# dfm/tinygp

Hardware: AMD Instinct MI355X
Metric: GP log_probability evals/sec + Cholesky TFLOP/s (fp64), N=16,384 (higher is better)
Workload: dtype f64; 1 GPU; c2: 1.5^2 ExpSquared(2.5), 1-D X, N=16384, fp64, diag=0.01, constant-density synthetic inputs (SURVEY 8d), dense Cholesky + tri-solve; n=16384, d=1, parallelism=single, nb_outer=1024

## Files before the change

### tinygp_amd/csrc/capi.hip

```cpp
#include <cmath>
#include <cstdlib>
#include <chrono>
#include <cstring>
#include <string>

#include "tgp_common.h"
#define CHAIN_HD __host__ __device__
#include "chain_tasks.h"
#define TILE_HD
#include "tile_order.h"

namespace tgp {

static thread_local std::string g_error;

void set_error(const char* fmt, ...) {
  char buf[1024];
  va_list ap;
  va_start(ap, fmt);
  vsnprintf(buf, sizeof(buf), fmt, ap);
  va_end(ap);
  g_error = buf;
}

// ... 155 lines not shown
  TGP_HIP_TRY(hipStreamCreateWithPriority(&ctx->update_stream, hipStreamNonBlocking, hi));
  TGP_HIP_TRY(hipStreamCreateWithPriority(&ctx->asm_stream, hipStreamNonBlocking, lo));
  TGP_HIP_TRY(hipEventCreateWithFlags(&ctx->ev_asm, hipEventDisableTiming));
  TGP_HIP_TRY(hipEventCreateWithFlags(&ctx->ev_d, hipEventDisableTiming));
  TGP_HIP_TRY(hipEventCreateWithFlags(&ctx->ev_e, hipEventDisableTiming));
  TGP_HIP_TRY(hipEventCreateWithFlags(&ctx->ev_f, hipEventDisableTiming));
  TGP_HIP_TRY(hipEventCreateWithFlags(&ctx->ev_g1, hipEventDisableTiming));
  TGP_HIP_TRY(hipEventCreateWithFlags(&ctx->ev_g2, hipEventDisableTiming));
  TGP_HIP_TRY(hipEventCreateWithFlags(&ctx->ev_h, hipEventDisableTiming));
  TGP_HIP_TRY(hipEventCreateWithFlags(&ctx->ev_i, hipEventDisableTiming));
  TGP_HIP_TRY(hipEventCreateWithFlags(&ctx->ev_j, hipEventDisableTiming));
  TGP_HIP_TRY(hipEventCreateWithFlags(&ctx->ev_c, hipEventDisableTiming));
  TGP_HIP_TRY(hipEventCreateWithFlags(&ctx->ev_join, hipEventDisableTiming));
  TGP_HIP_TRY(hipEventCreateWithFlags(&ctx->ev_a, hipEventDisableTiming));
  TGP_HIP_TRY(hipEventCreateWithFlags(&ctx->ev_b, hipEventDisableTiming));
  TGP_HIP_TRY(hipMalloc(&ctx->d_scal, 16 * sizeof(double)));
  TGP_HIP_TRY(hipMalloc(&ctx->d_info, sizeof(int32_t)));
  TGP_HIP_TRY(hipMalloc(&ctx->d_step_flag, 64));
  TGP_HIP_TRY(hipMemset(ctx->d_step_flag, 0, 64));
  TGP_HIP_TRY(hipMalloc(&ctx->d_chain_flags, size_t(tgp::CHAIN_MAX_ROW_TILES) * 64 * sizeof(uint32_t)));
  TGP_HIP_TRY(hipMemset(ctx->d_chain_flags, 0, size_t(tgp::CHAIN_MAX_ROW_TILES) * 64 * sizeof(uint32_t)));
  TGP_HIP_TRY(hipMalloc(&ctx->d_chain_ticket, 4096));
  TGP_HIP_TRY(hipMemset(ctx->d_chain_ticket, 0, 4096));
  TGP_HIP_TRY(hipMalloc(&ctx->d_chain_red, size_t(2) * CHAIN_MAX_ROW_TILES * sizeof(double)));
  hipDeviceProp_t prop;
  TGP_HIP_TRY(hipGetDeviceProperties(&prop, device));
  ctx->cus = prop.multiProcessorCount;
  *out = ctx;
  return TGP_OK;
}

int tgp_ctx_destroy(tgp_ctx* ctx) {
// ... 17 lines not shown
    hipStreamSynchronize(ctx->asm_stream);
    hipStreamDestroy(ctx->asm_stream);
  }
  if (ctx->ev_asm) hipEventDestroy(ctx->ev_asm);
  if (ctx->ev_d) hipEventDestroy(ctx->ev_d);
  if (ctx->ev_e) hipEventDestroy(ctx->ev_e);
  if (ctx->ev_f) hipEventDestroy(ctx->ev_f);
  if (ctx->ev_g1) hipEventDestroy(ctx->ev_g1);
  if (ctx->ev_g2) hipEventDestroy(ctx->ev_g2);
  if (ctx->ev_h) hipEventDestroy(ctx->ev_h);
  if (ctx->ev_i) hipEventDestroy(ctx->ev_i);
  if (ctx->ev_j) hipEventDestroy(ctx->ev_j);
  for (auto e : ctx->ev_pool) hipEventDestroy(e);
  if (ctx->ev_a) hipEventDestroy(ctx->ev_a);
  if (ctx->ev_b) hipEventDestroy(ctx->ev_b);
  if (ctx->d_scal) hipFree(ctx->d_scal);
  if (ctx->d_info) hipFree(ctx->d_info);
  if (ctx->d_step_flag) hipFree(ctx->d_step_flag);
  if (ctx->d_chain_flags) hipFree(ctx->d_chain_flags);
  if (ctx->d_chain_ticket) hipFree(ctx->d_chain_ticket);
  if (ctx->d_chain_red) hipFree(ctx->d_chain_red);
  if (ctx->d_chain_stamps) hipFree(ctx->d_chain_stamps);
  for (auto& kv : ctx->chain_tables)
    if (kv.second.dev) hipFree(kv.second.dev);
  if (ctx->d_dinv) hipFree(ctx->d_dinv);
  if (ctx->d_work) hipFree(ctx->d_work);
  if (ctx->d_gemm_ws) hipFree(ctx->d_gemm_ws);
  if (ctx->d_gemm_prefix_count) hipFree(ctx->d_gemm_prefix_count);
  if (ctx->panel_stream) hipStreamDestroy(ctx->panel_stream);
  if (ctx->own_stream && ctx->stream) hipStreamDestroy(ctx->stream);
  delete ctx;
  return TGP_OK;
// ... 398 lines not shown
    tgp_ctx* ctx = s->ctx;
    for (hipStream_t q : {ctx->asm_stream, ctx->panel_stream, ctx->update_stream, ctx->solve_stream, ctx->stream})
      if (q) (void)hipStreamSynchronize(q);
    (void)hipGetLastError();
    ctx->asm_pending = false;
    ctx->deferred_asm = nullptr;
    ctx->ev_used = 0;
    ctx->timeout_retries++;
    const int64_t keep = ctx->chain_kernel;
    ctx->chain_kernel = 0;
    st = factor_body(s, prog, nops, cov_host, info, fused, resid_host, logprob);
    ctx->chain_kernel = keep;
  }
  if (st < 0) {
    tgp_ctx* ctx = s->ctx;
    ctx->asm_pending = false;
    ctx->deferred_asm = nullptr;
    ctx->ev_used = 0;
    s->factored = false;
    for (hipStream_t q : {ctx->asm_stream, ctx->panel_stream, ctx->update_stream, ctx->solve_stream,
                          ctx->stream})
      if (q) (void)hipStreamSynchronize(q);
    (void)hipGetLastError();
  }
  return st;
}

static int factor_body(tgp_solver* s, const tgp_kop* prog, int nops, const void* cov_host,
                       int32_t* info, int fused, const void* resid_host, double* logprob) {
  tgp_ctx* ctx = s->ctx;
// ... 6 lines not shown
  TGP_ARG_CHECK(s->has_prog || cov_host != nullptr, "factor needs a kernel program or a covariance");
  s->winv_valid = false;
  const auto host0 = std::chrono::steady_clock::now();
  const size_t es = esize(s->dtype);
  hipEvent_t e0 = nullptr, e1 = nullptr, e2 = nullptr;
  const bool prof = ctx->profile != 0;
  if (prof) {
    TGP_HIP_TRY(hipEventCreate(&e0));
    TGP_HIP_TRY(hipEventCreate(&e1));
    TGP_HIP_TRY(hipEventCreate(&e2));
    TGP_HIP_TRY(hipEventRecord(e0, ctx->stream));
  }
  int status = dispatch(s->dtype, [&](auto tag) {
    using T = decltype(tag);
    T* A = (T*)s->A;
    if (fused) {
      if (resid_host) {
        TGP_TRY(upload_vec(s, s->vec, resid_host));
      } else {
        TGP_ARG_CHECK(s->has_resid, "no resident residual: call tgp_solver_set_resid first");
        TGP_HIP_TRY(hipMemcpyAsync(s->vec, s->resid, size_t(s->npad) * es, hipMemcpyDeviceToDevice,
                                   ctx->stream));
      }
    }
    if (cov_host != nullptr) {
      TGP_TRY(solver_scratch(s, size_t(s->n) * s->n * es));
      TGP_HIP_TRY(hipMemcpyAsync(s->scratch, cov_host, size_t(s->n) * s->n * es,
                                 hipMemcpyHostToDevice, ctx->stream));
      TGP_TRY(launch_set_lower_from_rowmajor<T>(ctx, s->n, s->npad, (const T*)s->scratch, A, s->npad));
    } else {
      TGP_TRY(assemble_lower<T>(ctx, s->kp, s->n, s->d, (const T*)s->X, (const T*)s->diag, A, s->npad));
    }
    if (prof) TGP_HIP_TRY(hipEventRecord(e1, ctx->stream));
    int32_t inf = 0;
    ctx->defer_join = ctx->late_join != 0;
    ctx->join_deferred = false;
    reductions_begin(ctx, s->npad, fused != 0);
    int st = potrf<T>(ctx, s->npad, A, s->npad, (T*)s->dinv, &inf, fused ? (T*)s->vec : (T*)nullptr);
    ctx->defer_join = false;
    const bool reduce = reductions_end(ctx);
    if (st < 0) return st;
    s->info = inf;
    if (prof) TGP_HIP_TRY(hipEventRecord(e2, ctx->stream));
    if (reduce) {
      TGP_TRY(launch_sum_log_diag<T>(ctx, s->n, A, s->npad, 1));
      if (fused) TGP_TRY(launch_sum_squares<T>(ctx, s->n, (const T*)s->vec, 0));
    }
    return TGP_OK;
  });
  if (status < 0) return status;
  double two[2] = {0, 0};
  int32_t inf_late = 0;
  const bool late = ctx->join_deferred;
  ctx->join_deferred = false;
  TGP_HIP_TRY(hipMemcpyAsync(two, ctx->d_scal, 2 * sizeof(double), hipMemcpyDeviceToHost, ctx->stream));
  if (late) TGP_HIP_TRY(hipMemcpyAsync(&inf_late, ctx->d_info, sizeof(int32_t), hipMemcpyDeviceToHost, ctx->stream));
  TGP_HIP_TRY(hipStreamSynchronize(ctx->stream));
  if (late) {
    if (inf_late == INT32_MIN) {
      tgp::set_error("potrf: a device-side hand-off did not arrive within poll_timeout_ms (a lost or starved chain launch)");
      if (prof) { hipEventDestroy(e0); hipEventDestroy(e1); hipEventDestroy(e2); }
      return TGP_E_TIMEOUT;
    }
    s->info = inf_late;
  }
  s->ms[5] = std::chrono::duration<double, std::milli>(ctx->submitted - host0).count();
  s->logdet_half = two[1];
  if (fused && logprob)
    *logprob = -0.5 * two[0] - (s->logdet_half + 0.5 * double(s->n) * std::log(2.0 * M_PI));
  if (prof) {
    float a = 0, b = 0;
    TGP_HIP_TRY(hipEventElapsedTime(&a, e0, e1));
// ... 563 lines not shown
```

### tinygp_amd/csrc/chol.hip

```cpp
#include <algorithm>
#include <atomic>
#include <functional>
#include <type_traits>

#include <thread>

#include "tgp_common.h"
#define CHAIN_HD __host__ __device__
#include "chain_tasks.h"

namespace tgp {

namespace {

typedef double d4 __attribute__((ext_vector_type(4)));
typedef float f4 __attribute__((ext_vector_type(4)));

template <typename T> struct Mfma;
template <> struct Mfma<double> {
  using acc_t = d4;
  static __device__ __forceinline__ acc_t mma(double a, double b, acc_t c) {
    return __builtin_amdgcn_mfma_f64_16x16x4f64(a, b, c, 0, 0, 0);
  }
  static __device__ __forceinline__ int drow(int lane, int r) { return (lane >> 4) + 4 * r; }
// ... 58 lines not shown
#ifdef TGP_POTF2_STAMPS
__device__ long long g_potf2_stamps[64];
#define POTF2_STAMP(i) do { if (threadIdx.x == 0) g_potf2_stamps[i] = __builtin_readcyclecounter(); } while (0)
#else
#define POTF2_STAMP(i) do {} while (0)
#endif

__device__ void potf2_prefix_wait(const int32_t* count, int32_t target, int32_t* info);

template <typename T, bool FOLD>
__global__ __launch_bounds__(512) __attribute__((amdgpu_waves_per_eu(4, 4))) void potf2_kernel(T* __restrict__ A, int64_t ld,
                                                    T* __restrict__ dinv,
                                                    int32_t* __restrict__ info,
                                                    int32_t pivot_base,
                                                    const T* __restrict__ Xp, int64_t ldx,
                                                    const int32_t* __restrict__ wait_count, int32_t wait_target) {
  __shared__ __attribute__((aligned(16))) T S[36 * 256];
  __shared__ T Rs[2 * 16];
  __shared__ T Dg[256];
  if (wait_count != nullptr) {
    if (threadIdx.x == 0) potf2_prefix_wait(wait_count, wait_target, info);
    __syncthreads();
  }
#include "potf2_body.inc"
}

constexpr int32_t STEP_TIMEOUT = INT32_MIN;

__device__ long long g_poll_limit = 400000000LL;
struct PollClock {
  long long t0 = 0;
  __device__ __forceinline__ bool expired(long spin) {
    if ((spin & 255) != 255) return false;
    const long long now = (long long)__builtin_amdgcn_s_memrealtime();
// ... 276 lines not shown
    }
    if (lane == 0) __builtin_amdgcn_fence(__ATOMIC_ACQUIRE, "agent");
  }
  __syncthreads();
}

__device__ __forceinline__ void chain_publish(uint32_t* word, uint32_t value, int32_t* colcnt = nullptr) {
  asm volatile("s_waitcnt vmcnt(0)" ::: "memory");
  __syncthreads();
  if (threadIdx.x == 0) {
    __hip_atomic_store(word, value, __ATOMIC_RELAXED, __HIP_MEMORY_SCOPE_AGENT);
    if (colcnt != nullptr) __hip_atomic_fetch_add(colcnt, 1, __ATOMIC_RELAXED, __HIP_MEMORY_SCOPE_AGENT);
  }
}

__device__ void potf2_prefix_wait(const int32_t* count, int32_t target, int32_t* info) {
  PollClock clk;
  for (unsigned spin = 0;; ++spin) {
    if (__hip_atomic_load(count, __ATOMIC_RELAXED, __HIP_MEMORY_SCOPE_AGENT) >= target) break;
    __builtin_amdgcn_s_sleep(8);
    if ((spin & 255) == 255 && (clk.expired(spin) || poisoned(info))) {
      atomicExch(info, STEP_TIMEOUT);
      break;
    }
  }
  __builtin_amdgcn_fence(__ATOMIC_ACQUIRE, "agent");
}

__global__ __launch_bounds__(64) void chain_poll_kernel(const int32_t* __restrict__ count, int32_t target,
                                                        int32_t* __restrict__ info) {
  if (threadIdx.x != 0) return;
  PollClock clk;
  for (unsigned spin = 0;; ++spin) {
    if (__hip_atomic_load(count, __ATOMIC_RELAXED, __HIP_MEMORY_SCOPE_AGENT) >= target) break;
    __builtin_amdgcn_s_sleep(16);
    if ((spin & 255) == 255 && (clk.expired(spin) || poisoned(info))) {
      atomicExch(info, STEP_TIMEOUT);
      break;
    }
  }
}

template <typename T, int PARTS>
__device__ __forceinline__ void chain_update_full(const ChainArgs<T>& q, T* S, int i, int c, int k, int part) {
  static_assert(PARTS == 1 || PARTS == 4 || PARTS == 8, "whole tile, row quarters or row eighths");
  using M = Mfma<T>;
  using acc_t = typename M::acc_t;
  typedef T T2 __attribute__((ext_vector_type(2)));
  const int tid = threadIdx.x, lane = tid & 63;
// ... 1566 lines not shown
    if ((spin & 63) != 63) continue;
    const double ms = std::chrono::duration<double, std::milli>(std::chrono::steady_clock::now() - t0).count();
    if (ms > budget_ms) break;
    if (ms > 50.0) std::this_thread::sleep_for(std::chrono::microseconds(200));
  }
  if (ctx->rescue_stream == nullptr) TGP_HIP_TRY(hipStreamCreateWithFlags(&ctx->rescue_stream, hipStreamNonBlocking));
  for (int c = 0; c < CHAIN_FLAG_LD; ++c)
    (void)hipStreamWriteValue32(ctx->rescue_stream, ctx->d_chain_ticket + CHAIN_COLCNT_OFF + c, 0x7fffffffu, 0);
  for (hipStream_t q : {ctx->rescue_stream, ctx->asm_stream, ctx->panel_stream, ctx->update_stream, ctx->solve_stream, ctx->stream})
    if (q) (void)hipStreamSynchronize(q);
  (void)hipGetLastError();
  set_error("potrf: the followers of a chain launch were still waiting after %.0f ms (stream wait-values released by the host)", budget_ms);
  return TGP_E_TIMEOUT;
}

template <typename T>
int launch_potf2(tgp_ctx* ctx, hipStream_t st, T* A, int64_t ld, T* dinv, int32_t* info,
                 int32_t pivot_base, const T* Xp, int64_t ldx) {
  if (ctx->trace) {
    trace_push(ctx, 1, st, trace_off(ctx, A), trace_off(ctx, Xp), ld);
    return TGP_OK;
  }
  const int32_t* wc = ctx->potf2_wait_counter;
  const int32_t wt = (int32_t)ctx->potf2_wait_target;
  ctx->potf2_wait_counter = nullptr;
  if (Xp != nullptr)
    hipLaunchKernelGGL((potf2_kernel<T, true>), dim3(1), dim3(512), 0, st, A, ld, dinv, info, pivot_base, Xp, ldx, wc, wt);
  else
    hipLaunchKernelGGL((potf2_kernel<T, false>), dim3(1), dim3(512), 0, st, A, ld, dinv, info, pivot_base, Xp, ldx, wc, wt);
  TGP_HIP_TRY(hipGetLastError());
  return TGP_OK;
}

template <typename T>
int launch_trsm(tgp_ctx* ctx, hipStream_t st, int64_t m, const T* L, int64_t ldl, const T* dinv,
                T* B, int64_t ldb) {
  if (m == 0) return TGP_OK;
  TGP_ARG_CHECK(m % 16 == 0, "trsm: m must be a multiple of 16");
  if (ctx->trace) {
    trace_push(ctx, 2, st, trace_off(ctx, L), trace_off(ctx, B), m, ldl);
    return TGP_OK;
  }
  hipLaunchKernelGGL((trsm_kernel<T>), dim3((unsigned)((m + 63) / 64)), dim3(256), 0, st, m, L,
                     ldl, dinv, B, ldb);
  TGP_HIP_TRY(hipGetLastError());
// ... 20 lines not shown
  TGP_HIP_TRY(hipGetLastError());
  return TGP_OK;
}

template <typename T>
ChainPolicy chain_policy(const tgp_ctx* ctx) {
  if (sizeof(T) != 8 || ctx->chain_batch <= 1) return ChainPolicy{1, 1, 2, 0};
  return ChainPolicy{(int)ctx->chain_batch, (int)ctx->chain_batch_lag, (int)ctx->chain_batch_rowlag, (int)ctx->chain_batch_minrows};
}

template <typename T>
int launch_chain(tgp_ctx* ctx, hipStream_t st, T* A0, int64_t ld, T* dinv0, int64_t pivot_base, int64_t R,
                 int64_t nblk, int64_t cb, int64_t ce, bool head_done, hipEvent_t counters_ready, T* y0, bool fprev) {
  TGP_ARG_CHECK(R >= 1 && R <= CHAIN_MAX_ROW_TILES && cb >= 0 && cb < ce && ce <= nblk && nblk <= CHAIN_FLAG_LD && nblk <= R,
                "chain: bad panel shape (R=%lld, columns [%lld, %lld))", (long long)R, (long long)cb, (long long)ce);
  if (cb == 0 && !head_done) {
    TGP_TRY(launch_potf2<T>(ctx, st, A0, ld, dinv0, ctx->d_info, (int32_t)pivot_base));
    if (!ctx->trace) TGP_TRY(run_deferred_asm(ctx, st));
  }
  if (ctx->chain_polls_pending) {
    TGP_TRY(st_wait(ctx, st, ctx->ev_f));
    ctx->chain_polls_pending = false;
  }
  const int fwd = y0 != nullptr ? 1 : 0;
  int red = 0;
  if (fwd != 0 && ctx->chain_red_total > 0 && ctx->chain_red_total <= CHAIN_MAX_ROW_TILES && pivot_base % TILE == 0) {
    red = 1;
    ctx->chain_red_written += ce - cb;
    if (pivot_base / TILE + ce == ctx->chain_red_total && ctx->chain_red_written == ctx->chain_red_total) {
      red = 2;
      ctx->reductions_done = true;
    }
  }
  if (ctx->trace) {
    if (counters_ready != nullptr) TGP_TRY(ev_record(ctx, counters_ready, st));
    trace_push(ctx, 11, st, trace_off(ctx, A0), ld, R, cb, ce, nblk, fwd, red);
    return TGP_OK;
  }
// ... 29 lines not shown
  q.launch = (int32_t)ctx->chain_launches++;
  q.fast_update = (int32_t)ctx->chain_fast_update;
  q.tasks = found->second.dev;
  q.y = y0;
  q.fgs = CHAIN_FWD_GROUP;
  q.fprev = fprev ? 1 : 0;
  q.red = red != 0 ? ctx->d_chain_red : nullptr;
  q.scal = red != 0 ? ctx->d_scal : nullptr;
  q.red_total = red == 2 ? (int32_t)ctx->chain_red_total : 0;
  if (ctx->chain_stamps != 0 && ctx->chain_stamp_base + tasks <= CHAIN_STAMP_TASKS) {
    if (ctx->d_chain_stamps == nullptr)
      TGP_HIP_TRY(hipMalloc((void**)&ctx->d_chain_stamps, size_t(CHAIN_STAMP_TASKS) * 16 * sizeof(long long)));
    q.stamps = ctx->d_chain_stamps + ctx->chain_stamp_base * 16;
    ctx->chain_stamp_base += tasks;
  }
  TGP_HIP_TRY(hipMemsetAsync(ctx->d_chain_ticket, 0, size_t(CHAIN_TICKET_WORDS) * sizeof(int32_t), st));
  if (counters_ready != nullptr) TGP_TRY(ev_record(ctx, counters_ready, st));
  const size_t dyn = ctx->chain_lds_pad > 0 ? size_t(ctx->chain_lds_pad) + (sizeof(T) == 4 ? 36 * 256 * 4 : 0) : 0;
  hipLaunchKernelGGL((chain_kernel<T>), dim3((unsigned)tasks), dim3(512), dyn, st, q);
  TGP_HIP_TRY(hipGetLastError());
  return TGP_OK;
}

int launch_chain_poll(tgp_ctx* ctx, hipStream_t st, const void* A0, int64_t ld, int64_t R, int64_t c, bool first_external) {
  if (ctx->trace) {
    trace_push(ctx, 12, st, trace_off(ctx, static_cast<const double*>(A0)), ld, c);
    return TGP_OK;
  }
  const int32_t target = (int32_t)(R - c - ((c == 0 && first_external) ? 1 : 0));
  int32_t* count = ctx->d_chain_ticket + CHAIN_COLCNT_OFF + c;
  if (ctx->chain_polls == 3 && ctx->can_wait_value) {
// ... 190 lines not shown
  if (n == 0) return TGP_OK;
  ctx->potf2_wait_counter = nullptr;
  ctx->prefix_hint_cols = 0;
  ctx->prefix_hint_counter = nullptr;
  ctx->reserve_hint = 0;
  hipStream_t S0 = ctx->stream, S1 = ctx->panel_stream;
  if (ctx->solve_on_update == 0 && y != nullptr) TGP_TRY(ensure_solve_stream(ctx));
  hipStream_t S2 = ctx->solve_on_update != 0 ? ctx->update_stream : ctx->solve_stream;
  if (y != nullptr) {
    TGP_TRY(ev_record(ctx, ctx->ev_c, S0));
    TGP_TRY(st_wait(ctx, S2, ctx->ev_c));
  }
  int64_t NB = ctx->nb_outer;
  if (NB < TILE) NB = TILE;
  NB = NB / TILE * TILE;
  if (!ctx->trace) TGP_HIP_TRY(hipMemsetAsync(ctx->d_info, 0, sizeof(int32_t), S0));
  ctx->chain_stamp_base = 0;
  ctx->chain_launches = 0;
  ctx->chain_polls_pending = false;
  const bool prof_on = ctx->profile != 0 && !ctx->trace;
  std::vector<ProfSpan> spans;
  ctx->ev_used = 0;
  hipEvent_t prof_t0 = nullptr;
  const bool span_dump = prof_on && getenv("TGP_SPAN_DUMP") != nullptr;
  if (prof_on) {
    TGP_TRY(prof_event(ctx, &prof_t0));
    TGP_HIP_TRY(hipEventRecord(prof_t0, S0));
  }

  auto potf2_at = [&](hipStream_t st, int64_t j0, bool pend) -> int {
    return panel_potf2<T>(ctx, st, A, ld, dinv, 0, j0, pend);
// ... 33 lines not shown
    const int64_t rem = n - k0;
    int64_t w = NB;
    if (k0 == 0 && ctx->nb_first >= TILE) w = ctx->nb_first / TILE * TILE;
    if (ctx->nb_wide_rows > 0 && k0 > 0 && rem >= ctx->nb_wide_rows) w = 2 * NB;
    if (ctx->chain_kernel != 0 && rem <= ctx->chain_full_rows && rem / TILE <= 64) w = rem;
    return rem < w ? rem : w;
  };
  bool all_chain = ctx->chain_kernel != 0;
  for (int64_t k0 = 0; k0 < n && all_chain; k0 += width(k0))
    all_chain = width(k0) / TILE <= CHAIN_FLAG_LD && (n - k0) / TILE <= CHAIN_MAX_ROW_TILES;
  ctx->chain_fwd_now = y != nullptr && ctx->chain_fwd_tasks != 0 && all_chain;
  auto chain_of_panel = [&](hipStream_t st, int64_t k0, int64_t w) -> int {
    const int64_t sp = ctx->chain_sub_panel / TILE * TILE;
    if (sp >= TILE && sp < w && w % sp == 0 && n - k0 > w && n - k0 >= ctx->chain_sub_min_rows) {
      for (int64_t o = 0; o < w; o += sp) {
        if (o > 0) TGP_TRY(potf2_at(st, k0 + o, false));
        TGP_TRY(panel(st, k0 + o, sp, true, 0, no_mid));
        const int64_t c0 = k0 + o + sp;
        if (c0 < k0 + w)
          TGP_TRY(trailing(st, n - c0, k0 + w - c0, sp, A + (k0 + o) * ld + c0, A + c0 * ld + c0, (int)ctx->chain_sub_role));
      }
      return TGP_OK;
    }
    return panel(st, k0, w, true, 0, no_mid);
  };
  const bool la = ctx->lookahead != 0 && S1 != nullptr;
  if (la && ctx->chain_kernel != 0 && ctx->chain_merged != 0) {
    std::vector<int64_t> s0;
    for (int64_t k0 = 0; k0 < n; k0 += width(k0)) s0.push_back(k0);
    s0.push_back(n);
    const int64_t P = (int64_t)s0.size() - 1;
// ... 5 lines not shown
      TGP_TRY(run_deferred_asm(ctx, nullptr));
    } else {
    TGP_TRY(ev_record(ctx, ctx->ev_a, S0));
    TGP_TRY(st_wait(ctx, S1, ctx->ev_a));
    TGP_TRY(panel(S1, 0, s0[1] - s0[0], false, 0, no_mid));
    TGP_TRY(run_deferred_asm(ctx, nullptr));
    TGP_TRY(ev_record(ctx, ev_chain[0], S1));
    for (int64_t p = 0; p + 1 < P; ++p) {
      const int64_t kb = s0[p + 1] - s0[p], next = s0[p + 1], wn = s0[p + 2] - s0[p + 1], mt = n - next;
      const T* Pp = A + s0[p] * ld + next;
      T* C = A + next * ld + next;
      TGP_TRY(st_wait(ctx, S0, ev_chain[p & 1]));
      if (p == 0 && asm_side) TGP_TRY(st_wait(ctx, S0, ctx->ev_asm));
      const bool prefix = wn < mt && ctx->chain_polls != 0;
      int32_t* counter = ctx->d_chain_ticket + CHAIN_PREFIX_OFF + (p & 3);
      if (prefix) {
        if (!ctx->trace) TGP_HIP_TRY(hipMemsetAsync(counter, 0, sizeof(int32_t), S0));
        TGP_TRY(ev_record(ctx, ev_pfx[p & 1], S0));
        ctx->prefix_hint_cols = wn;
        ctx->prefix_hint_counter = counter;
      }
      const int64_t t = mt / TILE;
      if (t * (t + 1) / 2 <= ctx->reserve_max_tiles) ctx->reserve_hint = ctx->chain_reserve;
      TGP_TRY(trailing(S0, mt, mt, kb, Pp, C, 0));
      if (!prefix) TGP_TRY(ev_record(ctx, ev_T[p & 1], S0));
      if (prefix) {
        const int64_t tm = mt / TILE, tp = wn / TILE;
        TGP_TRY(st_wait(ctx, S1, ev_pfx[p & 1]));
        if (ctx->trace || ctx->chain_polls == 2) {
          TGP_TRY(launch_prefix_poll(ctx, S1, counter, tp * tm - tp * (tp - 1) / 2, trace_off(ctx, C), ld));
        } else {
          ctx->potf2_wait_counter = counter;
          ctx->potf2_wait_target = tp * tm - tp * (tp - 1) / 2;
        }
      } else {
        TGP_TRY(st_wait(ctx, S1, ev_T[p & 1]));
      }
      if (p == 0 && asm_side) TGP_TRY(st_wait(ctx, S1, ctx->ev_asm));
      TGP_TRY(potf2_at(S1, next, false));
      TGP_TRY(chain_of_panel(S1, next, wn));
      TGP_TRY(ev_record(ctx, ev_chain[(p + 1) & 1], S1));
    }
    TGP_TRY(st_wait(ctx, S0, ev_chain[(P - 1) & 1]));
    }
  } else
  if (la && ctx->chain_kernel != 0 && ctx->chain_depth2 != 0) {
    std::vector<int64_t> s0;
    for (int64_t k0 = 0; k0 < n; k0 += width(k0)) s0.push_back(k0);
    s0.push_back(n);
    const int64_t P = (int64_t)s0.size() - 1;
    hipEvent_t ev_chain[2] = {ctx->ev_b, ctx->ev_g1}, ev_pre[2] = {ctx->ev_g2, ctx->ev_e};
    auto first_role = [&](int64_t m, int64_t nn) -> int {
      const int64_t tiles = (m / TILE) * (nn / TILE) - (nn / TILE) * (nn / TILE - 1) / 2;
// ... 188 lines not shown
    double hi = -1e300;
    for (const auto& q : iv) {
      if (q.first > hi) {
        ctx->prof_syrk_union_ms += q.second - q.first;
        hi = q.second;
      } else if (q.second > hi) {
        ctx->prof_syrk_union_ms += q.second - hi;
        hi = q.second;
      }
    }
  }
  if (info == STEP_TIMEOUT) {
    set_error("potrf: a device-side hand-off did not arrive within poll_timeout_ms (a lost or starved chain launch)");
    return TGP_E_TIMEOUT;
  }
  if (info_host) *info_host = info;
  return info > 0 ? info : TGP_OK;
}

template <typename T>
int compute_winv(tgp_ctx* ctx, int64_t n, const T* L, int64_t ld, T* winv) {
  if (n == 0) return TGP_OK;
  const int64_t sec = (n / TILE) * 16384;
  hipLaunchKernelGGL((winv_kernel<T>), dim3((unsigned)(n / TILE)), dim3(128), 0, ctx->stream, (int)(n / TILE), L, ld,
                     winv, winv + sec, winv + 2 * sec, winv + 3 * sec);
  TGP_HIP_TRY(hipGetLastError());
  return TGP_OK;
}

template <typename T>
// ... 239 lines not shown
```

### tinygp_amd/csrc/kmat.hip

```cpp
#include <algorithm>

#include "tgp_common.h"
#include "kprog_eval.h"

namespace tgp {

namespace {

constexpr int KT = 128;

template <typename T>
__device__ __forceinline__ void load_tile_pair(T* s1, T* s2, const T* __restrict__ X1, const T* __restrict__ X2,
                                               int64_t r0, int64_t c0, int64_t n1, int64_t n2, int d) {
  for (int t = threadIdx.x; t < KT * d; t += 256) {
    const int64_t gi = r0 + t / d, gj = c0 + t / d;
    s1[t] = (gi < n1) ? X1[gi * d + t % d] : T(0);
    s2[t] = (gj < n2) ? X2[gj * d + t % d] : T(0);
  }
  __syncthreads();
}

template <int NT, int NACC>
__device__ __forceinline__ void block_sum(double (&acc)[NACC]) {
  __shared__ double red[NACC][NT];
// ... 76 lines not shown
      const T a = MathC<T>::SQRT3 * by_p0.template div<FAST>(dist);
      return (T(1) + a) * exp(-a);
    } else {
      const T a = MathC<T>::SQRT5 * by_p0.template div<FAST>(dist);
      return (T(1) + a + by3.template div<FAST>(a * a)) * exp(-a);
    }
  }
}

template <typename T, int OP, int L2>
__device__ __forceinline__ T leaf_fast(T r1, T r2, T p0, T p0sq) {
  const UDiv<T> by_p0(p0), by_p0sq(p0sq), by3(T(3));
  return leaf_fast<T, OP, L2, false>(r1, r2, by_p0, by_p0sq, by3);
}

template <typename T, int D, int OP, int L2>
__global__ __launch_bounds__(256) void kmat_fast_kernel(T p0, T amp, int64_t n1, int64_t n2,
                                                        const T* __restrict__ X1,
                                                        const T* __restrict__ X2,
                                                        const T* __restrict__ diag, T* __restrict__ out,
                                                        int64_t ld, int flags, int tc0, int tri_h) {
  typedef T T2 __attribute__((ext_vector_type(2)));
  constexpr int NCOL = 32;
  const int cq = threadIdx.x >> 6, l = threadIdx.x & 63;
  int tr, tc;
  if (flags & KMAT_LOWER) {
    const int b = blockIdx.x;
    const double h2 = 2.0 * tri_h + 1.0;
    int j = int((h2 - sqrt(h2 * h2 - 8.0 * double(b))) * 0.5);
    while (j > 0 && j * tri_h - j * (j - 1) / 2 > b) --j;
    while ((j + 1) * tri_h - (j + 1) * j / 2 <= b) ++j;
    tc = tc0 + j;
    tr = tc + (b - (j * tri_h - j * (j - 1) / 2));
  } else {
    tr = blockIdx.x;
    tc = blockIdx.y + tc0;
  }
  __shared__ T s2all[KT * D];
// ... 42 lines not shown
    return seen;
  };
  bool plain = true;
  if (sizeof(T) == 8 && !(flags & KMAT_PLAIN_DIV) && by_p0.exact && by_p0sq.exact) {
    plain = !(columns(std::true_type{}) <= T(0x1p300));
  }
  if (plain) columns(std::false_type{});
}

template <typename T, int D, int FAM>
__global__ __launch_bounds__(256) void kmat_kernel(KProg kp, int64_t n1, int64_t n2, int d,
                                                   const T* __restrict__ X1,
                                                   const T* __restrict__ X2,
                                                   const T* __restrict__ diag, T* __restrict__ out,
                                                   int64_t ld, int64_t rows_out, int64_t cols_out,
                                                   int flags, int tc0, int ftr, int ftc) {
  const int tr = blockIdx.x, tc = blockIdx.y + tc0;
  if ((flags & KMAT_LOWER) && tr < tc) return;
  if (tr < ftr && tc < ftc) return;
  extern __shared__ __attribute__((aligned(16))) char smem[];
  T* s1 = reinterpret_cast<T*>(smem);
  T* s2 = s1 + KT * d;
  const int64_t r0 = int64_t(tr) * KT, c0 = int64_t(tc) * KT;
  load_tile_pair(s1, s2, X1, X2, r0, c0, n1, n2, d);

  const int il = threadIdx.x & (KT - 1);
  const int g = threadIdx.x >> 7;
  const int64_t gi = r0 + il;
  T xr[D > 0 ? D : 1];
  if constexpr (D > 0) {
#pragma unroll
    for (int t = 0; t < D; ++t) xr[t] = s1[il * D + t];
// ... 325 lines not shown

template <typename T>
int launch_kmat_cols(tgp_ctx* ctx, hipStream_t st, const KProg& kp, int64_t n1, int64_t n2, int d,
                     const T* X1, const T* X2, const T* diag, T* out, int64_t ld, int64_t rows_out,
                     int64_t cols_out, int flags, int64_t tc0, int64_t ntc) {
  TGP_ARG_CHECK(d >= 1 && d <= TGP_MAX_DIM, "input dimension must be 1..%d (got %d)", TGP_MAX_DIM, d);
  TGP_ARG_CHECK(rows_out >= n1 && cols_out >= n2 && ld >= rows_out, "kmat: bad output extents");
  if (rows_out == 0 || cols_out == 0 || ntc <= 0) return TGP_OK;
  const int64_t tr = (rows_out + KT - 1) / KT, tc = (cols_out + KT - 1) / KT;
  TGP_ARG_CHECK(tc0 >= 0 && tc0 + ntc <= tc, "kmat: column tile range outside the matrix");
  if (ctx->trace) {
    trace_push(ctx, 7, st, tc0, ntc, ld, flags);
    return TGP_OK;
  }
  TGP_ARG_CHECK(ntc <= 65535, "kmat: too many column tiles");
  int ftr = 0, ftc = 0;
  const FastProg fp = fast_prog(kp);
  if (fp.op >= 0 && d <= 3 && ld % 2 == 0 && reinterpret_cast<uintptr_t>(out) % 16 == 0) {
    ftr = int(n1 / KT);
    ftc = int(n2 / KT);
    const int64_t fc = std::min<int64_t>(tc0 + ntc, ftc) - tc0;
    const int64_t tri_h = (flags & KMAT_LOWER) ? ftr - tc0 : 0;
    const int64_t tri_c = std::min<int64_t>(fc, tri_h);
    const bool any = (flags & KMAT_LOWER) ? (tri_c > 0) : (ftr > 0 && fc > 0);
    if (any) {
      dim3 fgrid((unsigned)ftr, (unsigned)fc);
      if (flags & KMAT_LOWER) fgrid = dim3((unsigned)(tri_c * tri_h - tri_c * (tri_c - 1) / 2));
      const int fflags = flags | (ctx->kmat_plain_div != 0 ? KMAT_PLAIN_DIV : 0);
      with_dim<3>(d, [&](auto dd) {
        with_fast_leaf(fp, [&](auto op, auto l2) {
          constexpr int D = decltype(dd)::value, OP = decltype(op)::value, L2 = decltype(l2)::value;
          hipLaunchKernelGGL((kmat_fast_kernel<T, D, OP, L2>), fgrid, dim3(256), 0, st, T(fp.p0), T(fp.amp), n1, n2, X1,
                             X2, diag, out, ld, fflags, (int)tc0, (int)tri_h);
        });
      });
    } else {
      ftr = ftc = 0;
    }
    if (ftr == tr && ftc >= tc0 + ntc) {
      TGP_HIP_TRY(hipGetLastError());
      return TGP_OK;
    }
  }
  dim3 grid((unsigned)tr, (unsigned)ntc);
  const size_t shmem = 2 * size_t(KT) * d * sizeof(T);
  with_dim<4>(d, [&](auto dd) {
    with_family<true>(kp, [&](auto fam) {
      constexpr int D = decltype(dd)::value, FAM = decltype(fam)::value;
      hipLaunchKernelGGL((kmat_kernel<T, D, FAM>), grid, dim3(256), shmem, st, kp, n1, n2, d, X1, X2, diag, out, ld,
                         rows_out, cols_out, flags, (int)tc0, ftr, ftc);
    });
  });
  TGP_HIP_TRY(hipGetLastError());
  return TGP_OK;
}

template <typename T>
int launch_kmat(tgp_ctx* ctx, const KProg& kp, int64_t n1, int64_t n2, int d, const T* X1,
                const T* X2, const T* diag, T* out, int64_t ld, int64_t rows_out, int64_t cols_out,
                int flags) {
  return launch_kmat_cols<T>(ctx, ctx->stream, kp, n1, n2, d, X1, X2, diag, out, ld, rows_out,
                             cols_out, flags, 0, (cols_out + KT - 1) / KT);
}

template <typename T>
int launch_kdiag(tgp_ctx* ctx, const KProg& kp, int64_t n, int d, const T* X, const T* add, T* out) {
  if (n == 0) return TGP_OK;
  const dim3 grid((unsigned)((n + 255) / 256));
// ... 156 lines not shown
```

### tinygp_amd/csrc/tgp_common.h

```cpp
#pragma once

#include <hip/hip_runtime.h>

#include <cstdarg>
#include <cstdint>
#include <cstdio>
#include <chrono>
#include <array>
#include <functional>
#include <map>
#include <mutex>
#include <vector>

#include "../../include/tgp_hip.h"

namespace tgp {

constexpr int TILE = TGP_TILE;
constexpr int SUB = 16;

void set_error(const char* fmt, ...);

#define TGP_HIP_TRY(expr)                                                                  \
  do {                                                                                     \
// ... 83 lines not shown
  int64_t gemm_prefix_count = 0;
  int32_t* d_gemm_prefix_count = nullptr;
  int64_t late_join = 1;
  int64_t chain_reduce = 1;
  double* d_chain_red = nullptr;
  int64_t chain_red_total = 0;
  int64_t chain_red_written = 0;
  bool reductions_done = false;
  bool defer_join = false;
  bool join_deferred = false;
  int64_t reserve_hint = 0;
  int64_t prefix_hint_cols = 0;
  int32_t* prefix_hint_counter = nullptr;
  const int32_t* potf2_wait_counter = nullptr;
  int64_t potf2_wait_target = 0;
  uint32_t* d_step_flag = nullptr;
  uint32_t step_epoch = 0;
  int64_t chain_kernel = 1;
  uint32_t* d_chain_flags = nullptr;
  int32_t* d_chain_ticket = nullptr;
  int64_t chain_fast_update = 0;
  int64_t chain_batch = 1;
  int64_t chain_batch_lag = 1;
  int64_t chain_batch_rowlag = 4;
  int64_t chain_batch_minrows = 32;
  struct ChainTable {
    uint64_t* dev = nullptr;
    int64_t count = 0;
  };
  std::map<std::array<int64_t, 9>, ChainTable> chain_tables;
// ... 256 lines not shown
```

Before: 39.92 evals/s.

## Fold small memsets and copies into kernels, use monotonic prefix counters

```diff
diff --git a/tinygp_amd/csrc/capi.hip b/tinygp_amd/csrc/capi.hip
--- a/tinygp_amd/csrc/capi.hip
+++ b/tinygp_amd/csrc/capi.hip
@@ -193,8 +193,9 @@
   TGP_HIP_TRY(hipEventCreateWithFlags(&ctx->ev_join, hipEventDisableTiming));
   TGP_HIP_TRY(hipEventCreateWithFlags(&ctx->ev_a, hipEventDisableTiming));
   TGP_HIP_TRY(hipEventCreateWithFlags(&ctx->ev_b, hipEventDisableTiming));
-  TGP_HIP_TRY(hipMalloc(&ctx->d_scal, 16 * sizeof(double)));
-  TGP_HIP_TRY(hipMalloc(&ctx->d_info, sizeof(int32_t)));
+  TGP_HIP_TRY(hipMalloc(&ctx->d_info, 16 + 16 * sizeof(double)));
+  ctx->d_scal = reinterpret_cast<double*>(reinterpret_cast<char*>(ctx->d_info) + 16);
+  TGP_HIP_TRY(hipHostMalloc(&ctx->h_ret, 32, hipHostMallocDefault));
   TGP_HIP_TRY(hipMalloc(&ctx->d_step_flag, 64));
   TGP_HIP_TRY(hipMemset(ctx->d_step_flag, 0, 64));
   TGP_HIP_TRY(hipMalloc(&ctx->d_chain_flags, size_t(tgp::CHAIN_MAX_ROW_TILES) * 64 * sizeof(uint32_t)));
@@ -242,8 +243,8 @@
   for (auto e : ctx->ev_pool) hipEventDestroy(e);
   if (ctx->ev_a) hipEventDestroy(ctx->ev_a);
   if (ctx->ev_b) hipEventDestroy(ctx->ev_b);
-  if (ctx->d_scal) hipFree(ctx->d_scal);
   if (ctx->d_info) hipFree(ctx->d_info);
+  if (ctx->h_ret) hipHostFree(ctx->h_ret);
   if (ctx->d_step_flag) hipFree(ctx->d_step_flag);
   if (ctx->d_chain_flags) hipFree(ctx->d_chain_flags);
   if (ctx->d_chain_ticket) hipFree(ctx->d_chain_ticket);
@@ -672,6 +673,7 @@
   }
   if (st < 0) {
     tgp_ctx* ctx = s->ctx;
+    ctx->info_zeroed = false;
     ctx->asm_pending = false;
     ctx->deferred_asm = nullptr;
     ctx->ev_used = 0;
@@ -708,13 +710,14 @@
   int status = dispatch(s->dtype, [&](auto tag) {
     using T = decltype(tag);
     T* A = (T*)s->A;
+    const bool resid_in_asm = fused && !resid_host && cov_host == nullptr;
     if (fused) {
       if (resid_host) {
         TGP_TRY(upload_vec(s, s->vec, resid_host));
       } else {
         TGP_ARG_CHECK(s->has_resid, "no resident residual: call tgp_solver_set_resid first");
-        TGP_HIP_TRY(hipMemcpyAsync(s->vec, s->resid, size_t(s->npad) * es, hipMemcpyDeviceToDevice,
-                                   ctx->stream));
+        if (!resid_in_asm)
+          TGP_HIP_TRY(hipMemcpyAsync(s->vec, s->resid, size_t(s->npad) * es, hipMemcpyDeviceToDevice, ctx->stream));
       }
     }
     if (cov_host != nullptr) {
@@ -723,7 +726,16 @@
                                  hipMemcpyHostToDevice, ctx->stream));
       TGP_TRY(launch_set_lower_from_rowmajor<T>(ctx, s->n, s->npad, (const T*)s->scratch, A, s->npad));
     } else {
-      TGP_TRY(assemble_lower<T>(ctx, s->kp, s->n, s->d, (const T*)s->X, (const T*)s->diag, A, s->npad));
+      ctx->asm_zero_info = true;
+      ctx->asm_copy_src = resid_in_asm ? s->resid : nullptr;
+      ctx->asm_copy_dst = resid_in_asm ? s->vec : nullptr;
+      ctx->asm_copy_n = resid_in_asm ? s->npad : 0;
+      const int ast = assemble_lower<T>(ctx, s->kp, s->n, s->d, (const T*)s->X, (const T*)s->diag, A, s->npad);
+      ctx->asm_zero_info = false;
+      ctx->asm_copy_n = 0;
+      TGP_TRY(ast);
+      if (resid_in_asm && !ctx->info_zeroed)
+        TGP_HIP_TRY(hipMemcpyAsync(s->vec, s->resid, size_t(s->npad) * es, hipMemcpyDeviceToDevice, ctx->stream));
     }
     if (prof) TGP_HIP_TRY(hipEventRecord(e1, ctx->stream));
     int32_t inf = 0;
@@ -747,9 +759,11 @@
   int32_t inf_late = 0;
   const bool late = ctx->join_deferred;
   ctx->join_deferred = false;
-  TGP_HIP_TRY(hipMemcpyAsync(two, ctx->d_scal, 2 * sizeof(double), hipMemcpyDeviceToHost, ctx->stream));
-  if (late) TGP_HIP_TRY(hipMemcpyAsync(&inf_late, ctx->d_info, sizeof(int32_t), hipMemcpyDeviceToHost, ctx->stream));
+  TGP_HIP_TRY(hipMemcpyAsync(ctx->h_ret, ctx->d_info, 32, hipMemcpyDeviceToHost, ctx->stream));
   TGP_HIP_TRY(hipStreamSynchronize(ctx->stream));
+  memcpy(&inf_late, ctx->h_ret, sizeof(int32_t));
+  memcpy(two, static_cast<const char*>(ctx->h_ret) + 16, sizeof(two));
+  if (late && inf_late == 0) ctx->counters_open = false;
   if (late) {
     if (inf_late == INT32_MIN) {
       tgp::set_error("potrf: a device-side hand-off did not arrive within poll_timeout_ms (a lost or starved chain launch)");
diff --git a/tinygp_amd/csrc/chol.hip b/tinygp_amd/csrc/chol.hip
--- a/tinygp_amd/csrc/chol.hip
+++ b/tinygp_amd/csrc/chol.hip
@@ -96,10 +96,14 @@
                                                     int32_t* __restrict__ info,
                                                     int32_t pivot_base,
                                                     const T* __restrict__ Xp, int64_t ldx,
-                                                    const int32_t* __restrict__ wait_count, int32_t wait_target) {
+                                                    const int32_t* __restrict__ wait_count, int32_t wait_target,
+                                                    int32_t* __restrict__ zero_words, int32_t zero_count) {
   __shared__ __attribute__((aligned(16))) T S[36 * 256];
   __shared__ T Rs[2 * 16];
   __shared__ T Dg[256];
+  if (zero_words != nullptr)
+    for (int t = threadIdx.x; t < zero_count; t += 512)
+      __hip_atomic_store(zero_words + t, 0, __ATOMIC_RELAXED, __HIP_MEMORY_SCOPE_AGENT);
   if (wait_count != nullptr) {
     if (threadIdx.x == 0) potf2_prefix_wait(wait_count, wait_target, info);
     __syncthreads();
@@ -406,10 +410,14 @@
   }
 }
 
+__device__ __forceinline__ bool count_reached(int32_t count, int32_t target) {
+  return int32_t(uint32_t(count) - uint32_t(target)) >= 0;
+}
+
 __device__ void potf2_prefix_wait(const int32_t* count, int32_t target, int32_t* info) {
   PollClock clk;
   for (unsigned spin = 0;; ++spin) {
-    if (__hip_atomic_load(count, __ATOMIC_RELAXED, __HIP_MEMORY_SCOPE_AGENT) >= target) break;
+    if (count_reached(__hip_atomic_load(count, __ATOMIC_RELAXED, __HIP_MEMORY_SCOPE_AGENT), target)) break;
     __builtin_amdgcn_s_sleep(8);
     if ((spin & 255) == 255 && (clk.expired(spin) || poisoned(info))) {
       atomicExch(info, STEP_TIMEOUT);
@@ -424,7 +432,7 @@
   if (threadIdx.x != 0) return;
   PollClock clk;
   for (unsigned spin = 0;; ++spin) {
-    if (__hip_atomic_load(count, __ATOMIC_RELAXED, __HIP_MEMORY_SCOPE_AGENT) >= target) break;
+    if (count_reached(__hip_atomic_load(count, __ATOMIC_RELAXED, __HIP_MEMORY_SCOPE_AGENT), target)) break;
     __builtin_amdgcn_s_sleep(16);
     if ((spin & 255) == 255 && (clk.expired(spin) || poisoned(info))) {
       atomicExch(info, STEP_TIMEOUT);
@@ -2021,6 +2029,21 @@
   return TGP_E_TIMEOUT;
 }
 
+constexpr uint32_t PREFIX_REFRESH = 1u << 30;
+int reset_counters(tgp_ctx* ctx, uint32_t start) {
+  for (hipStream_t q : {ctx->asm_stream, ctx->panel_stream, ctx->update_stream, ctx->solve_stream, ctx->stream})
+    if (q) TGP_HIP_TRY(hipStreamSynchronize(q));
+  uint32_t words[4] = {start, start, start, start};
+  TGP_HIP_TRY(hipMemsetAsync(ctx->d_chain_ticket, 0, 4096, ctx->stream));
+  TGP_HIP_TRY(hipMemcpyAsync(ctx->d_chain_ticket + CHAIN_PREFIX_OFF, words, sizeof(words), hipMemcpyHostToDevice, ctx->stream));
+  TGP_HIP_TRY(hipStreamSynchronize(ctx->stream));
+  for (int q = 0; q < 4; ++q) ctx->prefix_base[q] = start;
+  ctx->ticket_zeroed_on = nullptr;
+  ctx->potf2_zero_ticket = false;
+  ctx->counters_open = false;
+  return TGP_OK;
+}
+
 template <typename T>
 int launch_potf2(tgp_ctx* ctx, hipStream_t st, T* A, int64_t ld, T* dinv, int32_t* info,
                  int32_t pivot_base, const T* Xp, int64_t ldx) {
@@ -2031,11 +2054,17 @@
   const int32_t* wc = ctx->potf2_wait_counter;
   const int32_t wt = (int32_t)ctx->potf2_wait_target;
   ctx->potf2_wait_counter = nullptr;
+  int32_t* zw = ctx->potf2_zero_ticket ? ctx->d_chain_ticket : nullptr;
+  ctx->potf2_zero_ticket = false;
+  ctx->ticket_zeroed_on = nullptr;
   if (Xp != nullptr)
-    hipLaunchKernelGGL((potf2_kernel<T, true>), dim3(1), dim3(512), 0, st, A, ld, dinv, info, pivot_base, Xp, ldx, wc, wt);
+    hipLaunchKernelGGL((potf2_kernel<T, true>), dim3(1), dim3(512), 0, st, A, ld, dinv, info, pivot_base, Xp, ldx, wc, wt, zw,
+                       CHAIN_TICKET_WORDS);
   else
-    hipLaunchKernelGGL((potf2_kernel<T, false>), dim3(1), dim3(512), 0, st, A, ld, dinv, info, pivot_base, Xp, ldx, wc, wt);
+    hipLaunchKernelGGL((potf2_kernel<T, false>), dim3(1), dim3(512), 0, st, A, ld, dinv, info, pivot_base, Xp, ldx, wc, wt, zw,
+                       CHAIN_TICKET_WORDS);
   TGP_HIP_TRY(hipGetLastError());
+  if (zw != nullptr) ctx->ticket_zeroed_on = st;
   return TGP_OK;
 }
 
@@ -2086,7 +2115,9 @@
                  int64_t nblk, int64_t cb, int64_t ce, bool head_done, hipEvent_t counters_ready, T* y0, bool fprev) {
   TGP_ARG_CHECK(R >= 1 && R <= CHAIN_MAX_ROW_TILES && cb >= 0 && cb < ce && ce <= nblk && nblk <= CHAIN_FLAG_LD && nblk <= R,
                 "chain: bad panel shape (R=%lld, columns [%lld, %lld))", (long long)R, (long long)cb, (long long)ce);
+  const bool had_pollers = ctx->chain_polls_pending;
   if (cb == 0 && !head_done) {
+    ctx->potf2_zero_ticket = !ctx->trace && !had_pollers;
     TGP_TRY(launch_potf2<T>(ctx, st, A0, ld, dinv0, ctx->d_info, (int32_t)pivot_base));
     if (!ctx->trace) TGP_TRY(run_deferred_asm(ctx, st));
   }
@@ -2094,6 +2125,9 @@
     TGP_TRY(st_wait(ctx, st, ctx->ev_f));
     ctx->chain_polls_pending = false;
   }
+  const bool ticket_zero = ctx->ticket_zeroed_on != nullptr && ctx->ticket_zeroed_on == st && cb == 0 && !had_pollers;
+  ctx->ticket_zeroed_on = nullptr;
+  ctx->potf2_zero_ticket = false;
   const int fwd = y0 != nullptr ? 1 : 0;
   int red = 0;
   if (fwd != 0 && ctx->chain_red_total > 0 && ctx->chain_red_total <= CHAIN_MAX_ROW_TILES && pivot_base % TILE == 0) {
@@ -2153,7 +2187,7 @@
     q.stamps = ctx->d_chain_stamps + ctx->chain_stamp_base * 16;
     ctx->chain_stamp_base += tasks;
   }
-  TGP_HIP_TRY(hipMemsetAsync(ctx->d_chain_ticket, 0, size_t(CHAIN_TICKET_WORDS) * sizeof(int32_t), st));
+  if (!ticket_zero) TGP_HIP_TRY(hipMemsetAsync(ctx->d_chain_ticket, 0, size_t(CHAIN_TICKET_WORDS) * sizeof(int32_t), st));
   if (counters_ready != nullptr) TGP_TRY(ev_record(ctx, counters_ready, st));
   const size_t dyn = ctx->chain_lds_pad > 0 ? size_t(ctx->chain_lds_pad) + (sizeof(T) == 4 ? 36 * 256 * 4 : 0) : 0;
   hipLaunchKernelGGL((chain_kernel<T>), dim3((unsigned)tasks), dim3(512), dyn, st, q);
@@ -2374,7 +2408,22 @@
   int64_t NB = ctx->nb_outer;
   if (NB < TILE) NB = TILE;
   NB = NB / TILE * TILE;
-  if (!ctx->trace) TGP_HIP_TRY(hipMemsetAsync(ctx->d_info, 0, sizeof(int32_t), S0));
+  const bool info_zeroed = ctx->info_zeroed;
+  ctx->info_zeroed = false;
+  if (!ctx->trace && !info_zeroed) TGP_HIP_TRY(hipMemsetAsync(ctx->d_info, 0, sizeof(int32_t), S0));
+  ctx->potf2_zero_ticket = false;
+  ctx->ticket_zeroed_on = nullptr;
+  if (!ctx->trace) {
+    const uint32_t top = std::max(std::max(ctx->prefix_base[0], ctx->prefix_base[1]), std::max(ctx->prefix_base[2], ctx->prefix_base[3]));
+    if (ctx->fault_inject == 2 || ctx->fault_inject == 3) {
+      const uint32_t start = (ctx->fault_inject == 2 ? PREFIX_REFRESH : 0x80000000u) - 8u;
+      ctx->fault_inject = 0;
+      TGP_TRY(reset_counters(ctx, start));
+    } else if (ctx->counters_open || top >= PREFIX_REFRESH) {
+      TGP_TRY(reset_counters(ctx, 0));
+    }
+    ctx->counters_open = true;
+  }
   ctx->chain_stamp_base = 0;
   ctx->chain_launches = 0;
   ctx->chain_polls_pending = false;
@@ -2438,7 +2487,10 @@
     const int64_t sp = ctx->chain_sub_panel / TILE * TILE;
     if (sp >= TILE && sp < w && w % sp == 0 && n - k0 > w && n - k0 >= ctx->chain_sub_min_rows) {
       for (int64_t o = 0; o < w; o += sp) {
-        if (o > 0) TGP_TRY(potf2_at(st, k0 + o, false));
+        if (o > 0) {
+          ctx->potf2_zero_ticket = !ctx->trace && !ctx->chain_polls_pending;
+          TGP_TRY(potf2_at(st, k0 + o, false));
+        }
         TGP_TRY(panel(st, k0 + o, sp, true, 0, no_mid));
         const int64_t c0 = k0 + o + sp;
         if (c0 < k0 + w)
@@ -2474,8 +2526,9 @@
       if (p == 0 && asm_side) TGP_TRY(st_wait(ctx, S0, ctx->ev_asm));
       const bool prefix = wn < mt && ctx->chain_polls != 0;
       int32_t* counter = ctx->d_chain_ticket + CHAIN_PREFIX_OFF + (p & 3);
+      const int64_t pfx_tiles = (wn / TILE) * (mt / TILE) - (wn / TILE) * (wn / TILE - 1) / 2;
+      const uint32_t pfx_target = ctx->prefix_base[p & 3] + (uint32_t)pfx_tiles;
       if (prefix) {
-        if (!ctx->trace) TGP_HIP_TRY(hipMemsetAsync(counter, 0, sizeof(int32_t), S0));
         TGP_TRY(ev_record(ctx, ev_pfx[p & 1], S0));
         ctx->prefix_hint_cols = wn;
         ctx->prefix_hint_counter = counter;
@@ -2483,20 +2536,21 @@
       const int64_t t = mt / TILE;
       if (t * (t + 1) / 2 <= ctx->reserve_max_tiles) ctx->reserve_hint = ctx->chain_reserve;
       TGP_TRY(trailing(S0, mt, mt, kb, Pp, C, 0));
+      if (prefix && !ctx->trace) ctx->prefix_base[p & 3] = pfx_target;
       if (!prefix) TGP_TRY(ev_record(ctx, ev_T[p & 1], S0));
       if (prefix) {
-        const int64_t tm = mt / TILE, tp = wn / TILE;
         TGP_TRY(st_wait(ctx, S1, ev_pfx[p & 1]));
         if (ctx->trace || ctx->chain_polls == 2) {
-          TGP_TRY(launch_prefix_poll(ctx, S1, counter, tp * tm - tp * (tp - 1) / 2, trace_off(ctx, C), ld));
+          TGP_TRY(launch_prefix_poll(ctx, S1, counter, (int32_t)pfx_target, trace_off(ctx, C), ld));
         } else {
           ctx->potf2_wait_counter = counter;
-          ctx->potf2_wait_target = tp * tm - tp * (tp - 1) / 2;
+          ctx->potf2_wait_target = (int32_t)pfx_target;
         }
       } else {
         TGP_TRY(st_wait(ctx, S1, ev_T[p & 1]));
       }
       if (p == 0 && asm_side) TGP_TRY(st_wait(ctx, S1, ctx->ev_asm));
+      ctx->potf2_zero_ticket = !ctx->trace && !ctx->chain_polls_pending;
       TGP_TRY(potf2_at(S1, next, false));
       TGP_TRY(chain_of_panel(S1, next, wn));
       TGP_TRY(ev_record(ctx, ev_chain[(p + 1) & 1], S1));
@@ -2715,6 +2769,7 @@
     set_error("potrf: a device-side hand-off did not arrive within poll_timeout_ms (a lost or starved chain launch)");
     return TGP_E_TIMEOUT;
   }
+  if (info == 0 && !ctx->trace) ctx->counters_open = false;
   if (info_host) *info_host = info;
   return info > 0 ? info : TGP_OK;
 }
diff --git a/tinygp_amd/csrc/kmat.hip b/tinygp_amd/csrc/kmat.hip
--- a/tinygp_amd/csrc/kmat.hip
+++ b/tinygp_amd/csrc/kmat.hip
@@ -114,14 +114,31 @@
   return leaf_fast<T, OP, L2, false>(r1, r2, by_p0, by_p0sq, by3);
 }
 
+template <typename T>
+struct AsmSide {
+  int32_t* zero_info = nullptr;
+  const T* src = nullptr;
+  T* dst = nullptr;
+  int64_t n = 0;
+};
+template <typename T>
+__device__ __forceinline__ void asm_side_work(const AsmSide<T>& e) {
+  const int64_t b = int64_t(blockIdx.y) * gridDim.x + blockIdx.x;
+  if (e.zero_info != nullptr && b == 0 && threadIdx.x == 0) *e.zero_info = 0;
+  const int64_t stride = int64_t(gridDim.x) * gridDim.y * blockDim.x;
+  for (int64_t i = b * blockDim.x + threadIdx.x; i < e.n; i += stride) e.dst[i] = e.src[i];
+}
+
 template <typename T, int D, int OP, int L2>
 __global__ __launch_bounds__(256) void kmat_fast_kernel(T p0, T amp, int64_t n1, int64_t n2,
                                                         const T* __restrict__ X1,
                                                         const T* __restrict__ X2,
                                                         const T* __restrict__ diag, T* __restrict__ out,
-                                                        int64_t ld, int flags, int tc0, int tri_h) {
+                                                        int64_t ld, int flags, int tc0, int tri_h,
+                                                        AsmSide<T> side) {
   typedef T T2 __attribute__((ext_vector_type(2)));
   constexpr int NCOL = 32;
+  asm_side_work(side);
   const int cq = threadIdx.x >> 6, l = threadIdx.x & 63;
   int tr, tc;
   if (flags & KMAT_LOWER) {
@@ -194,8 +211,10 @@
                                                    const T* __restrict__ X2,
                                                    const T* __restrict__ diag, T* __restrict__ out,
                                                    int64_t ld, int64_t rows_out, int64_t cols_out,
-                                                   int flags, int tc0, int ftr, int ftc) {
+                                                   int flags, int tc0, int ftr, int ftc,
+                                                   AsmSide<T> side) {
   const int tr = blockIdx.x, tc = blockIdx.y + tc0;
+  asm_side_work(side);
   if ((flags & KMAT_LOWER) && tr < tc) return;
   if (tr < ftr && tc < ftc) return;
   extern __shared__ __attribute__((aligned(16))) char smem[];
@@ -551,6 +570,15 @@
     return TGP_OK;
   }
   TGP_ARG_CHECK(ntc <= 65535, "kmat: too many column tiles");
+  AsmSide<T> side;
+  if (ctx->asm_zero_info && st == ctx->stream) {
+    side.zero_info = ctx->d_info;
+    side.src = static_cast<const T*>(ctx->asm_copy_src);
+    side.dst = static_cast<T*>(ctx->asm_copy_dst);
+    side.n = side.src != nullptr && side.dst != nullptr ? ctx->asm_copy_n : 0;
+  }
+  const bool side_on = side.zero_info != nullptr;
+  ctx->asm_zero_info = false;
   int ftr = 0, ftc = 0;
   const FastProg fp = fast_prog(kp);
   if (fp.op >= 0 && d <= 3 && ld % 2 == 0 && reinterpret_cast<uintptr_t>(out) % 16 == 0) {
@@ -568,9 +596,11 @@
         with_fast_leaf(fp, [&](auto op, auto l2) {
           constexpr int D = decltype(dd)::value, OP = decltype(op)::value, L2 = decltype(l2)::value;
           hipLaunchKernelGGL((kmat_fast_kernel<T, D, OP, L2>), fgrid, dim3(256), 0, st, T(fp.p0), T(fp.amp), n1, n2, X1,
-                             X2, diag, out, ld, fflags, (int)tc0, (int)tri_h);
+                             X2, diag, out, ld, fflags, (int)tc0, (int)tri_h, side);
         });
       });
+      if (side_on) ctx->info_zeroed = true;
+      side = AsmSide<T>{};
     } else {
       ftr = ftc = 0;
     }
@@ -585,10 +615,11 @@
     with_family<true>(kp, [&](auto fam) {
       constexpr int D = decltype(dd)::value, FAM = decltype(fam)::value;
       hipLaunchKernelGGL((kmat_kernel<T, D, FAM>), grid, dim3(256), shmem, st, kp, n1, n2, d, X1, X2, diag, out, ld,
-                         rows_out, cols_out, flags, (int)tc0, ftr, ftc);
+                         rows_out, cols_out, flags, (int)tc0, ftr, ftc, side);
     });
   });
   TGP_HIP_TRY(hipGetLastError());
+  if (side.zero_info != nullptr) ctx->info_zeroed = true;
   return TGP_OK;
 }
 
diff --git a/tinygp_amd/csrc/tgp_common.h b/tinygp_amd/csrc/tgp_common.h
--- a/tinygp_amd/csrc/tgp_common.h
+++ b/tinygp_amd/csrc/tgp_common.h
@@ -121,6 +121,16 @@
   int32_t* prefix_hint_counter = nullptr;
   const int32_t* potf2_wait_counter = nullptr;
   int64_t potf2_wait_target = 0;
+  uint32_t prefix_base[4] = {0, 0, 0, 0};
+  bool counters_open = false;
+  bool potf2_zero_ticket = false;
+  hipStream_t ticket_zeroed_on = nullptr;
+  bool asm_zero_info = false;
+  bool info_zeroed = false;
+  const void* asm_copy_src = nullptr;
+  void* asm_copy_dst = nullptr;
+  int64_t asm_copy_n = 0;
+  void* h_ret = nullptr;
   uint32_t* d_step_flag = nullptr;
   uint32_t step_epoch = 0;
   int64_t chain_kernel = 1;
```

After: 40.05 evals/s, median of 6. Within noise of the previous version (+0.3%).
